# lc700x/desktop2stereo

Hardware: AMD Instinct MI355X
Metric: stereo frames/sec @1080p DepthAnything-v2-ViT-B (higher is better)
Workload: dtype bf16; 1 GPU; DepthAnything-v2-vitb bf16, 1920x1080 uint8 RGB noise frames, batch 1 per GPU, Depth Resolution 518 (model input 294x518), Full-SBS uint8 output 3840x1080, pred; parallelism=frame-sharded dp1, no data-path collective (each rank generates its own frames)

## Files before the change

### desktop2stereo_amd/csrc/core.cpp

```cpp
#include "common.h"

#include <atomic>
#include <cstdlib>

namespace d2s {

static thread_local std::string g_err;

void set_error(const std::string& msg) { g_err = msg; }

int hip_fail(hipError_t err, const char* what, const char* file, int line) {
    g_err = std::string("HIP error ") + hipGetErrorName(err) + " (" + hipGetErrorString(err) + ") in " + what +
            " at " + file + ":" + std::to_string(line);
    return D2S_E_HIP;
}

int env_int(const char* name, int dflt) {
    const char* v = getenv(name);
    return v ? atoi(v) : dflt;
}

static std::atomic<int> g_env_gen{1};
int env_generation() { return g_env_gen.load(std::memory_order_relaxed); }
int EnvInt::get() {
    const uint32_t g = (uint32_t)env_generation();
    const uint64_t c = cached.load(std::memory_order_relaxed);
    if ((uint32_t)(c >> 32) == g) return (int)(uint32_t)c;
    const int val = env_int(name, dflt);
    cached.store(((uint64_t)g << 32) | (uint32_t)val, std::memory_order_relaxed);
    return val;
}

int device_cu_count() {
    static const int n = [] { hipDeviceProp_t p; int d = 0; (void)hipGetDevice(&d); return hipGetDeviceProperties(&p, d) == hipSuccess ? p.multiProcessorCount : 256; }();
    return n;
}

}

extern "C" int d2s_debug_lds_poison(void) {
#ifdef D2S_LDS_POISON
    return 1;
#else
    return 0;
#endif
}
extern "C" int d2s_debug_reload_env(void) { return d2s::g_env_gen.fetch_add(1) + 1; }
extern "C" const char* d2s_last_error(void) { return d2s::g_err.c_str(); }
extern "C" int d2s_version(void) { return 132; }
```

### desktop2stereo_amd/csrc/gemm.hip

```cpp
#include "gemm_epi.h"
#include "linear_site.h"
#include <cstdio>
#include <deque>
#include <vector>

namespace d2s {

__device__ u32x4 d2s_zero_page[4];

#ifdef D2S_GLDS_TIMING
__device__ unsigned long long glds_timing[4096 * 8];
#define GL_STAMP(SLOT) { if (threadIdx.x == 0 && blockIdx.y == 0 && blockIdx.x < 4096) glds_timing[blockIdx.x * 8 + (SLOT)] = wall_clock64(); }
#else
#define GL_STAMP(SLOT) {}
#endif

__device__ __forceinline__ u32x4 relu_frag(u32x4 v, int, fp8_t) { return v; }
__device__ __forceinline__ u32x4 relu_frag(u32x4 v, int, bx3_t) { return v; }
__device__ __forceinline__ u32x4 relu_frag(u32x4 v, int floor_bits, float) {
    f32x4 x = __builtin_bit_cast(f32x4, v);
    float f = floor_bits == 0 ? 0.f : -3.0e38f;
    x = __builtin_elementwise_max(x, (f32x4){f, f, f, f});
    return __builtin_bit_cast(u32x4, x);
}

template <int N> __device__ __forceinline__ void wait_vmcnt() { asm volatile("s_waitcnt vmcnt(%0)" ::"n"(N) : "memory"); }

template <int CPR> __device__ __forceinline__ int swz_row(int r) { return CPR == 8 ? ((r >> 1) & 7) : (CPR == 4 ? ((r >> 1) & 3) : (r & 15)); }

static_assert(sizeof(GemmA) + sizeof(GemmEpi) + 8 >= KERNARG_WARM_BYTES, "KERNARG_WARM reads past the kernarg segment");
template <typename T, int BM, int BN, int WM, int WN, int NS, int CPR, int STG = 0>
__global__ void __launch_bounds__(64 * WM * WN)
gemm_glds_kernel(const T* __restrict__ W, const void* a_ptr, long a_lda, int M, int N, int K, int Kpad, int xn, GemmA a, GemmEpi e) {
    static_assert(STG == 0 || STG == 2 || (STG == 1 && NS == 2), "the register-staged variant uses two LDS stages");
    constexpr bool LEAN = STG == 2;
    constexpr bool BX3 = std::is_same<T, bx3_t>::value;
    static_assert(!BX3 || CPR == 8, "bf16x3 units are laid out for 128-byte K tiles");
    constexpr int CE = Prec<T>::CE;
    constexpr int BK = CPR * CE;
    constexpr int RPI = 64 / CPR;
    constexpr int NW = WM * WN;
    constexpr int AI = BM / (RPI * NW), BI = BN / (RPI * NW);
    constexpr int LPT = AI + BI;
    constexpr int FM = BM / WM / 16, FN = BN / WN / 16;
    constexpr int PD = NS - 1;
    constexpr int STAGE = (BM + BN) * CPR;
    __shared__ __attribute__((aligned(16))) u32x4 lds[NS * STAGE];
    KERNARG_WARM(kaw_)
    if constexpr (STG != 2) { KERNARG_WARM_END(kaw_) }
    D2S_POISON_LDS(lds, NS * STAGE)

    const int tid = threadIdx.x, lane = tid & 63;
    const int wid = __builtin_amdgcn_readfirstlane(tid >> 6);
    const int wave_m = wid / WN, wave_n = wid % WN;
    int tm_, tn_;
    GL_STAMP(0)
    if (!tile_of_block(blockIdx.x, (M + BM - 1) / BM, (N + BN - 1) / BN, xn, tm_, tn_)) return;
    const int bm0 = tm_ * BM, bn0 = tn_ * BN;
    static_assert((RPI * NW) % 16 == 0, "row swizzle must be invariant across a thread's instructions");
    static_assert(BM % (RPI * NW) == 0 && BN % (RPI * NW) == 0 && BM % (16 * WM) == 0 && BN % (16 * WN) == 0, "tile must split evenly over the waves");
    const int lrow = wid * RPI + lane / CPR;
    const int src_chunk = (lane % CPR) ^ swz_row<CPR>(lrow);
    const T* zero = (const T*)d2s_zero_page;

    const T* arow[AI];
    int aiy[AI], aix[AI];
    bool aok[AI];
    if constexpr (!LEAN)
#pragma unroll
    for (int i = 0; i < AI; ++i) {
        int m = bm0 + i * NW * RPI + lrow;
        aok[i] = m < M;
        int mm = aok[i] ? m : 0;
        if (a.mode == A_PLAIN) { arow[i] = (const T*)a.ptr + (long)mm * a.lda; aiy[i] = aix[i] = 0; }
        else {
            int ox = mm % a.Wo, oy = (mm / a.Wo) % a.Ho, b = mm / (a.Wo * a.Ho);
            aiy[i] = oy * a.stride - 1; aix[i] = ox * a.stride - 1;
            arow[i] = (const T*)a.ptr + (long)b * a.Hi * a.Wi * a.C;
        }
    }
    const T* wrow = W + (long)(bn0 + lrow) * Kpad + src_chunk * CE;
    const float inv_c = a.mode == A_CONV3 ? 1.0f / (float)a.C : 0.f;
    constexpr int ES = (int)sizeof(T);
    const __amdgpu_buffer_rsrc_t rsA = __builtin_amdgcn_make_buffer_rsrc(uniform_ptr(a_ptr), 0, (unsigned)((long)M * a_lda * ES), 0x00020000);
    const __amdgpu_buffer_rsrc_t rsW = __builtin_amdgcn_make_buffer_rsrc(uniform_ptr(W), 0, (unsigned)((long)((N + 255) / 256 * 256) * Kpad * ES), 0x00020000);
    unsigned voA[AI], voW[BI];
    if constexpr (STG != 1) {
        if (LEAN || a.buf) {
#pragma unroll
            for (int i = 0; i < AI; ++i) {
                const int m = bm0 + i * NW * RPI + lrow;
                voA[i] = m < M ? (unsigned)((long)m * a_lda * ES) + (unsigned)(src_chunk * 16) : 0x80000000u;
            }
#pragma unroll
            for (int i = 0; i < BI; ++i) voW[i] = (unsigned)((long)(bn0 + lrow + RPI * NW * i) * Kpad * ES) + (unsigned)(src_chunk * 16);
        }
    }
#define D2S_ISSUE_BUF(KT)                                                                                        \
    {                                                                                                            \
        u32x4* st_ = lds + ((KT) % NS) * STAGE;                                                                  \
        const int so_ = ((KT) + kt0) * (BK * ES);                                                                \
        _Pragma("unroll") for (int i = 0; i < AI; ++i) lds_dma16(rsA, st_ + (i * NW + wid) * 64, voA[i], so_);    \
        _Pragma("unroll") for (int i = 0; i < BI; ++i) lds_dma16(rsW, st_ + BM * CPR + (i * NW + wid) * 64, voW[i], so_); \
    }

    if constexpr (LEAN) {
        constexpr int kt0 = 0;
        const int nkt_ = (K + BK - 1) / BK;
#pragma unroll
        for (int t = 0; t < PD; ++t)
            if (t < nkt_) D2S_ISSUE_BUF(t)
        KERNARG_WARM_END(kaw_)
    }

    u32x4 stg[1][STG == 1 ? LPT : 1];
#define D2S_MOVE(S, IDX, SRC, DST)                                                                                \
    do {                                                                                                         \
        if constexpr (STG == 1) stg[S][IDX] = *(const u32x4*)(SRC);                                                 \
        else __builtin_amdgcn_global_load_lds((const __attribute__((address_space(1))) void*)(SRC),             \
                                              (__attribute__((address_space(3))) void*)(DST), 16, 0, 0);         \
    } while (0)
#define D2S_ISSUE_TILE(KT, S)                                                                                    \
    {                                                                                                            \
        u32x4* st_ = lds + ((KT) % NS) * STAGE;                                                                  \
        const int k_ = ((KT) + kt0) * BK + src_chunk * CE;                                                       \
        if (a.mode == A_PLAIN) {                                                                                 \
            _Pragma("unroll") for (int i = 0; i < AI; ++i) {                                                     \
                const T* s_ = (aok[i] && k_ < K) ? arow[i] + k_ : zero;                                          \
                D2S_MOVE(S, i, s_, st_ + (i * NW + wid) * 64);                                                    \
            }                                                                                                    \
        } else {                                                                                                 \
            int tap_ = (int)(((float)k_ + 0.5f) * inv_c);                                                        \
            int c0_ = k_ - tap_ * a.C;                                                                           \
            int ky_ = tap_ / 3, kx_ = tap_ - ky_ * 3;                                                            \
            _Pragma("unroll") for (int i = 0; i < AI; ++i) {                                                     \
                int iy_ = aiy[i] + ky_, ix_ = aix[i] + kx_;                                                      \
                bool ok_ = aok[i] && k_ < K && iy_ >= 0 && iy_ < a.Hi && ix_ >= 0 && ix_ < a.Wi;                 \
                const T* s_ = ok_ ? arow[i] + ((long)iy_ * a.Wi + ix_) * a.C + c0_ : zero;                       \
                D2S_MOVE(S, i, s_, st_ + (i * NW + wid) * 64);                                                    \
            }                                                                                                    \
        }                                                                                                        \
        _Pragma("unroll") for (int i = 0; i < BI; ++i)                                                           \
            D2S_MOVE(S, AI + i, wrow + (long)(RPI * NW * i) * Kpad + ((KT) + kt0) * BK, st_ + BM * CPR + (i * NW + wid) * 64); \
    }
    const int bx_row = (lane / CPR) * CPR, bx_sw = swz_row<CPR>(lrow);
    const int bx_hi = (bx_row + (((src_chunk >> 1) * 2) ^ bx_sw)) * 2 + (src_chunk & 1);
    const int bx_lo = (bx_row + (((src_chunk >> 1) * 2 + 1) ^ bx_sw)) * 2 + (src_chunk & 1);
#define D2S_STORE_STG(KT, S)                                                                                     \
    {                                                                                                            \
        u32x4* st_ = lds + ((KT) % NS) * STAGE;                                                                  \
        if constexpr (BX3) {                                                                                     \
            _Pragma("unroll") for (int i = 0; i < AI; ++i) {                                                     \
                f32x4 x_ = __builtin_bit_cast(f32x4, stg[S][i]);                                                 \
                if (a.relu) x_ = __builtin_elementwise_max(x_, (f32x4){0.f, 0.f, 0.f, 0.f});                     \
                uint2 h_, l_;                                                                                    \
                bx3_split4(x_, h_, l_);                                                                          \
                uint2* s2_ = (uint2*)(st_ + (i * NW + wid) * 64);                                                \
                s2_[bx_hi] = h_; s2_[bx_lo] = l_;                                                                \
            }                                                                                                    \
        } else {                                                                                                 \
            _Pragma("unroll") for (int i = 0; i < AI; ++i) st_[(i * NW + wid) * 64 + lane] = stg[S][i];          \
        }                                                                                                        \
        _Pragma("unroll") for (int i = 0; i < BI; ++i) st_[BM * CPR + (i * NW + wid) * 64 + lane] = stg[S][AI + i]; \
    }

    f32x4 acc[FM][FN];
#pragma unroll
    for (int i = 0; i < FM; ++i)
#pragma unroll
        for (int j = 0; j < FN; ++j) acc[i][j] = (f32x4){0.f, 0.f, 0.f, 0.f};

    const int nkt_all = (K + BK - 1) / BK;
    const int ksplit = LEAN ? 1 : (e.ksplit > 1 ? e.ksplit : 1);
    const int kt0 = (int)(((long)nkt_all * blockIdx.y) / ksplit);
    const int nkt = (int)(((long)nkt_all * (blockIdx.y + 1)) / ksplit) - kt0;
    const int fr = lane & 15, fg = lane >> 4;
    constexpr bool LN_ON = WN > 1;
    constexpr int LNS = LN_ON ? 4 : 1;
    float2 lnp[FM][LNS];
    if (LN_ON && e.ln_stats) {
#pragma unroll
        for (int i = 0; i < FM; ++i) {
            const int m = bm0 + wave_m * (BM / WM) + i * 16 + fr;
#pragma unroll
            for (int q = 0; q < LNS; ++q) {
                const int sl = fg + 4 * q;
                lnp[i][q] = (m < M && sl < e.ln_slots) ? ((const float2*)e.ln_stats)[(long)sl * (e.ln_M ? e.ln_M : M) + m] : make_float2(0.f, 0.f);
            }
        }
    }
#define D2S_COMPUTE(KT, RELU)                                                                                    \
    {                                                                                                            \
        const u32x4* A_l = lds + ((KT) % NS) * STAGE + (wave_m * (BM / WM)) * CPR;                               \
        const u32x4* B_l = lds + ((KT) % NS) * STAGE + BM * CPR + (wave_n * (BN / WN)) * CPR;                    \
        if constexpr (BX3) {                                                                                     \
             \
            const int cu_ = 2 * BX3_UNIT(fg);                                                                    \
            u32x4 fbh[FN], fbl[FN];                                                                              \
            _Pragma("unroll") for (int j = 0; j < FN; ++j) {                                                     \
                int r = j * 16 + fr; fbh[j] = B_l[r * CPR + (cu_ ^ swz_row<CPR>(r))]; fbl[j] = B_l[r * CPR + ((cu_ + 1) ^ swz_row<CPR>(r))]; \
            }                                                                                                    \
            _Pragma("unroll") for (int i = 0; i < FM; ++i) {                                                     \
                int r = i * 16 + fr;                                                                             \
                const u32x4 fah = A_l[r * CPR + (cu_ ^ swz_row<CPR>(r))], fal = A_l[r * CPR + ((cu_ + 1) ^ swz_row<CPR>(r))]; \
                _Pragma("unroll") for (int j = 0; j < FN; ++j) mma_bx3(acc[i][j], fbh[j], fbl[j], fah, fal);     \
            }                                                                                                    \
        } else {                                                                                                 \
        _Pragma("unroll") for (int ks = 0; ks < CPR / 4; ++ks) {                                                 \
                             \
                                            \
            u32x4 fb[FN];                                                                                        \
            _Pragma("unroll") for (int j = 0; j < FN; ++j) {                                                     \
                int r = j * 16 + fr; fb[j] = B_l[r * CPR + ((ks * 4 + fg) ^ swz_row<CPR>(r))];                   \
            }                                                                                                    \
            _Pragma("unroll") for (int i = 0; i < FM; ++i) {                                                     \
                int r = i * 16 + fr;                                                                             \
                u32x4 fa = A_l[r * CPR + ((ks * 4 + fg) ^ swz_row<CPR>(r))];                                     \
                if (RELU) fa = relu_frag(fa, 0, T());                                                            \
                _Pragma("unroll") for (int j = 0; j < FN; ++j) mma_chunk(acc[i][j], fb[j], fa, T());             \
            }                                                                                                    \
        }                                                                                                        \
        }                                                                                                        \
    }
#define D2S_K_LOOP(RELU)                                                                                         \
    if constexpr (STG == 1) {                                                                                    \
        for (int kt = 0; kt < nkt; ++kt) {                                                                       \
            __syncthreads();               \
            if (kt + 1 < nkt) D2S_STORE_STG(kt + 1, 0)                                                           \
            if (kt + 2 < nkt) D2S_ISSUE_TILE(kt + 2, 0)                                                          \
            D2S_COMPUTE(kt, RELU)                                                                                \
        }                                                                                                        \
    } else {                                                                                                     \
        for (int kt = 0; kt < nkt; ++kt) {                                                                       \
                          \
            if (kt + PD - 1 < nkt) wait_vmcnt<(PD - 1) * LPT>();                                                 \
            else wait_vmcnt<0>();                                                                                \
            __builtin_amdgcn_s_barrier();                                                                        \
            if (kt + PD < nkt) D2S_ISSUE_TILE(kt + PD, 0)                                                        \
            D2S_COMPUTE(kt, RELU)                                                                                \
        }                                                                                                        \
    }
    bool done_buf = false;
    if constexpr (STG != 1) {
        if (LEAN || a.buf) {
            if constexpr (!LEAN) {
#pragma unroll
                for (int t = 0; t < PD; ++t)
                    if (t < nkt) D2S_ISSUE_BUF(t)
            }
            GL_STAMP(1)
            for (int kt = 0; kt < nkt; ++kt) {
                if (kt + PD - 1 < nkt) wait_vmcnt<(PD - 1) * LPT>();
                else wait_vmcnt<0>();
                __builtin_amdgcn_s_barrier();
                if (kt == 0) { GL_STAMP(2) }
                if (kt + PD < nkt) D2S_ISSUE_BUF(kt + PD)
                D2S_COMPUTE(kt, 0)
            }
            done_buf = true;
        }
    }
    if constexpr (!LEAN)
    if (!done_buf) {
    if constexpr (STG == 1) {
        if (nkt > 0) { D2S_ISSUE_TILE(0, 0) D2S_STORE_STG(0, 0) }
        if (nkt > 1) D2S_ISSUE_TILE(1, 0)
    } else {
#pragma unroll
        for (int t = 0; t < PD; ++t)
            if (t < nkt) D2S_ISSUE_TILE(t, 0)
    }
    if (a.relu) { D2S_K_LOOP(1) } else { D2S_K_LOOP(0) }
    }
    GL_STAMP(3)
#undef D2S_ISSUE_BUF
#undef D2S_K_LOOP
#undef D2S_COMPUTE
#undef D2S_ISSUE_TILE
#undef D2S_STORE_STG
#undef D2S_MOVE

    if constexpr (WN == 1) {
        if (e.map == MAP_HEAD) {
            static_for<FM>([&](auto ic) {
                constexpr int i = decltype(ic)::value;
                const int m = bm0 + wave_m * (BM / WM) + i * 16 + fr;
                float s = 0.f;
                static_for<FN>([&](auto jc) {
                    constexpr int j = decltype(jc)::value;
                    const int n0 = j * 16 + fg * 4;
                    if (n0 < N) {
                        float b[4], w[4];
                        load4(e.bias + n0, b); load4(e.scale + n0, w);
                        s += fmaxf(acc[i][j][0] + b[0], 0.f) * w[0] + fmaxf(acc[i][j][1] + b[1], 0.f) * w[1] +
                             fmaxf(acc[i][j][2] + b[2], 0.f) * w[2] + fmaxf(acc[i][j][3] + b[3], 0.f) * w[3];
                    }
                });
                s += __shfl_xor(s, 16);
                s += __shfl_xor(s, 32);
                if (fg == 0 && m < M) ((float*)e.out)[m] = head_activation(s + e.head_b3, e.head_max_depth);
            });
            return;
        }
    }

    float2 ln_s[FM];
    float ln_cs[FN][4];
    if (LN_ON && e.ln_csum) {
#pragma unroll
        for (int j = 0; j < FN; ++j) {
            const int n0 = bn0 + wave_n * (BN / WN) + j * 16 + fg * 4;
            if (n0 < N) load4(e.ln_csum + n0, ln_cs[j]);
            else { ln_cs[j][0] = ln_cs[j][1] = ln_cs[j][2] = ln_cs[j][3] = 0.f; }
        }
    }
    constexpr bool PRE = STG == 2 && FM * FN <= 8;
    EpiCols cols[PRE ? FN : 1];
    if constexpr (PRE) {
#pragma unroll
        for (int j = 0; j < FN; ++j) {
            const int n0 = bn0 + wave_n * (BN / WN) + j * 16 + fg * 4;
            if (n0 < N) epi_cols_load(e, n0, cols[j]);
        }
    }
    float pre[PRE ? FM : 1][PRE ? FN : 1][4];
    const bool pre_on = PRE && ksplit == 1 && epi_res1_ahead(e);
    if constexpr (PRE) {
        if (pre_on) {
            static_for<FM>([&](auto ic) {
                constexpr int i = decltype(ic)::value;
                const int m = bm0 + wave_m * (BM / WM) + i * 16 + fr;
                static_for<FN>([&](auto jc) {
                    constexpr int j = decltype(jc)::value;
                    const int n0 = bn0 + wave_n * (BN / WN) + j * 16 + fg * 4;
                    if (m < M && n0 < N) epi_res1_load<T>(e, m, n0, pre[i][j]);
                });
            });
        }
    }
    static_for<FM>([&](auto ic) {
        constexpr int i = decltype(ic)::value;
        const int m = bm0 + wave_m * (BM / WM) + i * 16 + fr;
        float s1 = 0.f, s2 = 0.f;
        float ln_mean = 0.f, ln_rstd = 1.f;
        if (LN_ON && e.ln_csum) {
            float t1 = (lnp[i][0].x + lnp[i][1 % LNS].x) + (lnp[i][2 % LNS].x + lnp[i][3 % LNS].x);
            float t2 = (lnp[i][0].y + lnp[i][1 % LNS].y) + (lnp[i][2 % LNS].y + lnp[i][3 % LNS].y);
            t1 += __shfl_xor(t1, 16); t2 += __shfl_xor(t2, 16);
            t1 += __shfl_xor(t1, 32); t2 += __shfl_xor(t2, 32);
            ln_mean = t1 / (float)e.ln_dim;
            ln_rstd = rsqrtf(fmaxf(t2 / (float)e.ln_dim - ln_mean * ln_mean, 0.f) + e.ln_eps);
        }
        if (m < M) {
            static_for<FN>([&](auto jc) {
                constexpr int j = decltype(jc)::value;
                const int n0 = bn0 + wave_n * (BN / WN) + j * 16 + fg * 4;
                if (n0 < N) {
                    float v[4] = {acc[i][j][0], acc[i][j][1], acc[i][j][2], acc[i][j][3]};
                    if (ksplit > 1) store4(e.part + ((long)blockIdx.y * M + m) * N + n0, v);
                    else {
                        const bool ln = LN_ON && e.ln_csum != nullptr;
                        if (ln) {
                            if (e.deq) { float q[4]; load4(e.deq + n0, q); v[0] *= q[0]; v[1] *= q[1]; v[2] *= q[2]; v[3] *= q[3]; }
                            v[0] = ln_rstd * (v[0] - ln_mean * ln_cs[j][0]); v[1] = ln_rstd * (v[1] - ln_mean * ln_cs[j][1]);
                            v[2] = ln_rstd * (v[2] - ln_mean * ln_cs[j][2]); v[3] = ln_rstd * (v[3] - ln_mean * ln_cs[j][3]);
                        }
                        epilogue_dispatch<T>(e, m, n0, v, ln, PRE && pre_on ? pre[PRE ? i : 0][PRE ? j : 0] : nullptr, PRE ? &cols[PRE ? j : 0] : nullptr);
                        s1 += (v[0] + v[1]) + (v[2] + v[3]);
                        s2 += (v[0] * v[0] + v[1] * v[1]) + (v[2] * v[2] + v[3] * v[3]);
                    }
                }
            });
        }
        if (LN_ON && e.stats_out) {
            s1 += __shfl_xor(s1, 16); s2 += __shfl_xor(s2, 16);
            s1 += __shfl_xor(s1, 32); s2 += __shfl_xor(s2, 32);
            ln_s[i] = make_float2(s1, s2);
        }
    });
    if (LN_ON && e.stats_out) {
        float2* red = (float2*)lds;
        __syncthreads();
#pragma unroll
        for (int i = 0; i < FM; ++i)
            if (fg == 0) red[wave_n * BM + wave_m * (BM / WM) + i * 16 + fr] = ln_s[i];
        __syncthreads();
        for (int r = tid; r < BM; r += 64 * NW) {
            float2 t = red[r];
            for (int w = 1; w < WN; ++w) { t.x += red[w * BM + r].x; t.y += red[w * BM + r].y; }
            if (bm0 + r < M) ((float2*)e.stats_out)[(long)(bn0 / BN) * M + bm0 + r] = t;
        }
    }
#ifdef D2S_GLDS_TIMING
    asm volatile("s_waitcnt vmcnt(0)" ::: "memory");
    GL_STAMP(4)
#endif
}

template <typename T>
__global__ void __launch_bounds__(256)
splitk_reduce_kernel(GemmEpi e, int M, int N) {
    long idx = (long)blockIdx.x * blockDim.x + threadIdx.x;
    int n4 = N >> 2;
    if (idx >= (long)M * n4) return;
    int m = (int)(idx / n4), n0 = (int)(idx % n4) * 4;
    float v[4] = {0.f, 0.f, 0.f, 0.f};
    for (int s = 0; s < e.ksplit; ++s) {
        float p[4];
        load4(e.part + ((long)s * M + m) * N + n0, p);
        v[0] += p[0]; v[1] += p[1]; v[2] += p[2]; v[3] += p[3];
    }
    epilogue_dispatch<T>(e, m, n0, v);
}

template <typename T, int BN, int WM, int WN, int NS = 2>
__global__ void __launch_bounds__(64 * WM * WN)
conv3_halo_kernel(GemmA a, const T* __restrict__ W, int M, int N, int K, int Kpad, GemmEpi e, int xn) {
    KERNARG_WARM(kaw_)
    KERNARG_WARM_END(kaw_)
    constexpr int CE = Prec<T>::CE, CPR = 8, BK = CPR * CE, PD = NS - 1;
    constexpr int TW = 16, TH = 8, BM = TH * TW, HWD = TW + 2, HPX = (TH + 2) * HWD;
    constexpr int HCPP = 16;
    constexpr int NW = WM * WN, RPI = 64 / CPR;
    constexpr int BI = BN / (RPI * NW);
    static_assert(BI >= 1 && BM % (WM * 16) == 0 && BN % (WN * 16) == 0, "bad tile split");
    constexpr int FM = BM / WM / 16, FN = BN / WN / 16;
    constexpr int STAGE = BN * CPR;
    __shared__ __attribute__((aligned(16))) u32x4 lds[NS * STAGE + HPX * HCPP];
    D2S_POISON_LDS(lds, NS * STAGE + HPX * HCPP)
    u32x4* const halo = lds + NS * STAGE;

    const int tid = threadIdx.x, lane = tid & 63;
    const int wid = __builtin_amdgcn_readfirstlane(tid >> 6);
    const int wave_m = wid / WN, wave_n = wid % WN;
    const int tiles_x = (a.Wo + TW - 1) / TW, tiles_y = (a.Ho + TH - 1) / TH;
    const int nimg = M / (a.Ho * a.Wo);
    int tm_, tn_;
    if (!tile_of_block(blockIdx.x, nimg * tiles_y * tiles_x, (N + BN - 1) / BN, xn, tm_, tn_)) return;
    const int b = tm_ / (tiles_y * tiles_x), ty0 = ((tm_ / tiles_x) % tiles_y) * TH, tx0 = (tm_ % tiles_x) * TW;
    const int bn0 = tn_ * BN;
    const int cpp = a.C / CE, smask = cpp - 1;

    const int lrow = wid * RPI + lane / CPR;
    const int src_chunk = (lane % CPR) ^ swz_row<CPR>(lrow);
    const T* wrow = W + (long)(bn0 + lrow) * Kpad + src_chunk * CE;
#define D2S_ISSUE_W(KT)                                                                                               \
    {                                                                                                                 \
        u32x4* st_ = lds + ((KT) % NS) * STAGE;                                                                       \
        _Pragma("unroll") for (int i = 0; i < BI; ++i)                                                                \
            __builtin_amdgcn_global_load_lds((const __attribute__((address_space(1))) void*)(wrow + (long)(RPI * NW * i) * Kpad + (KT) * BK), \
                                             (__attribute__((address_space(3))) void*)(st_ + (i * NW + wid) * 64), 16, 0, 0);              \
    }
    const int nkt = K / BK;
#pragma unroll
    for (int t = 0; t < PD; ++t)
        if (t < nkt) D2S_ISSUE_W(t)
    conv_halo_fill<T, 64 * NW, 3>(a, b, ty0, tx0, HWD, HPX, cpp, tid, halo,
        [&](int p, int c) { return p * cpp + (c ^ (p & smask)); },
        [&](u32x4 v) { return a.relu ? relu_frag(v, 0, T()) : v; });
    f32x4 acc[FM][FN];
#pragma unroll
    for (int i = 0; i < FM; ++i)
#pragma unroll
        for (int j = 0; j < FN; ++j) acc[i][j] = (f32x4){0.f, 0.f, 0.f, 0.f};
    const int kpt = cpp / CPR;
    const int fr = lane & 15, fg = lane >> 4;
    int tap = 0, sub = 0;
    for (int kt = 0; kt < nkt; ++kt) {
        if (kt + PD - 1 < nkt) asm volatile("s_waitcnt vmcnt(%0) lgkmcnt(0)" ::"n"((PD - 1) * BI) : "memory");
        else asm volatile("s_waitcnt vmcnt(0) lgkmcnt(0)" ::: "memory");
        __builtin_amdgcn_s_barrier();
        if (kt + PD < nkt) D2S_ISSUE_W(kt + PD)
        const int ky = tap / 3, kx = tap - ky * 3, cb = sub * CPR;
        const u32x4* B_l = lds + (kt % NS) * STAGE + (wave_n * (BN / WN)) * CPR;
#pragma unroll
        for (int ks = 0; ks < CPR / 4; ++ks) {
            u32x4 fb[FN];
#pragma unroll
            for (int j = 0; j < FN; ++j) { int r = j * 16 + fr; fb[j] = B_l[r * CPR + ((ks * 4 + fg) ^ swz_row<CPR>(r))]; }
#pragma unroll
            for (int i = 0; i < FM; ++i) {
                const int p = (wave_m * FM + i + ky) * HWD + fr + kx;
                const u32x4 fa = halo[p * cpp + ((cb + ks * 4 + fg) ^ (p & smask))];
#pragma unroll
                for (int j = 0; j < FN; ++j) mma_chunk(acc[i][j], fb[j], fa, T());
            }
        }
        if (++sub == kpt) { sub = 0; ++tap; }
    }
#undef D2S_ISSUE_W
    const int nb = bn0 + wave_n * (BN / WN) + fg * 4;
    EpiCols cols[FN];
#pragma unroll
    for (int j = 0; j < FN; ++j)
        if (nb + j * 16 < N) epi_cols_load(e, nb + j * 16, cols[j]);
    conv_tile_epilogue<T, FM, FN>(a, e, acc, cols, b, ty0 + wave_m * FM, tx0 + fr, nb, N);
}

static inline bool buf_eligible(const GemmA& a, int M, int N, int K, int Kpad, int bk, size_t es) {
    return a.mode == A_PLAIN && !a.relu && K % bk == 0 && (long)M * a.lda * (long)es < (1L << 31) && (long)gemm_npad(N) * Kpad * (long)es < (1L << 31);
}

constexpr int SPLITK_GRID = 128;

static inline bool splitk_wanted(const GemmEpi& e, long tiles, int K, int bk) {
    return e.part && e.part_elems > 0 && !e.stats_out && tiles < SPLITK_GRID && cdiv(K, bk) >= 24;
}

static bool gemm_deep() {
    static EnvInt deep{"D2S_GEMM_DEEP", 1};
    return deep.get() != 0;
}

enum { TY_BF16 = 1, TY_E4M3 = 2, TY_F32 = 4, TY_BX3 = 8, TY_BEF = TY_BF16 | TY_E4M3 | TY_F32, TY_ALL = TY_BEF | TY_BX3 };
#define GLDS_INSTANCES(X)                                                                                                        \
                                                                                                   \
    X(G_256128, TY_BEF, 256,128,4,2,3,8,0)                                                                                       \
    X(G_128, TY_BEF, 128,128,2,2,4,8,0)                                                                                          \
    X(G_64, TY_BEF, 64,64,2,2,4,8,0)                                                                                             \
                      \
    X(G_3264, TY_ALL, 32,64,2,2,4,8,0)                                                                                           \
                             \
    X(G_1281288, TY_ALL, 128,128,2,4,2,8,0)                                                \
    X(G_641288, TY_ALL, 64,128,2,4,2,8,0)                                                                     \
    X(G_64648, TY_ALL, 64,64,4,2,2,8,0)                                                                       \
    X(G_256648, TY_BEF, 256,64,8,1,2,8,0)                                                         \
    X(G_128324, TY_BEF, 128,32,4,1,2,8,0)                                                                  \
          \
    X(G_964, TY_ALL, 64,64,2,2,2,8,1)                                                                                            \
    X(G_91288, TY_ALL, 128,128,4,2,2,8,1)                                                            \
    X(G_912832, TY_ALL, 128,32,4,1,2,8,1)                                                         \
    X(G_9256648, TY_ALL, 256,64,8,1,2,8,1)                                                                 \
// ... 24 lines not shown

static constexpr int glds_codes[][2] = {{256128, G_256128}, {128, G_128}, {64, G_64}, {3264, G_3264}, {1281288, G_1281288},
                                        {641288, G_641288}, {64648, G_64648}, {256648, G_256648}, {128324, G_128324}, {964, G_964},
                                        {91288, G_91288}, {912832, G_912832}, {9256648, G_9256648}};
static constexpr struct { int code, alias, auto_of, inst; } bx3_codes[] = {
    {93264, 3264, 3264, G_93264}, {964, 64, 64648, G_964}, {964128, 0, 641288, G_964128}, {91288, 128, 1281288, G_91288},
    {912832, 0, 912832, G_912832}, {9256648, 0, 9256648, G_9256648}};

#define HALO_INSTANCES(X) X(H_64, 64,4,2,4) X(H_128, 128,2,4,2)
enum {
#define X(ID, ...) ID,
    HALO_INSTANCES(X)
#undef X
};
static constexpr struct { int BN, WM, WN, NS; } halo_cfg[] = {
#define X(ID, ...) {__VA_ARGS__},
    HALO_INSTANCES(X)
#undef X
};
static const char* const halo_names[][4] = {
#define X(ID, ...) {"conv3_halo_kernel<bf16," #__VA_ARGS__ ">", nullptr, "conv3_halo_kernel<f32," #__VA_ARGS__ ">", nullptr},
    HALO_INSTANCES(X)
#undef X
};

static inline int type_index(int precision) {
    return precision == D2S_PREC_BF16 ? 0 : (precision == D2S_PREC_FP8_OPERANDS ? 1 : (precision == D2S_PREC_BF16X3 ? 3 : 2));
}
template <typename T> constexpr int type_bit() {
    return std::is_same<T, bf16_t>::value ? TY_BF16 : std::is_same<T, fp8_t>::value ? TY_E4M3 : std::is_same<T, bx3_t>::value ? TY_BX3 : TY_F32;
}

static int plan_fail(GemmPlan& p, int rc, const char* msg) { p.error = msg; return rc; }
static int glds_inst_of(int code) {
    for (const auto& c : glds_codes) if (c[0] == code) return c[1];
    return -1;
}

static int plan_glds(int inst, int precision, int tile, const GemmA& a, int M, int N, int K, int Kpad, const GemmEpi& e, GemmPlan& p) {
    const GldsCfg& c = glds_cfg[inst];
    const int es = (int)elem_size(precision), bk = c.CPR * (16 / es);
    p.family = GEMM_GLDS; p.inst = inst; p.name = glds_names[inst][type_index(precision)]; p.tile = tile; p.block = 64 * c.WM * c.WN;
    p.xn = pick_xn(cdiv(M, c.BM), cdiv(N, c.BN), c.BN, Kpad, es, p.grid);
    const int nkt = cdiv(K, bk);
    int ks = 1;
    if (c.STG != 2 && e.part && e.part_elems > 0 && !e.stats_out && (int)p.grid < SPLITK_GRID && nkt >= 24) {
        ks = nkt / 6; if (ks > 16) ks = 16;
        while (ks > 1 && (size_t)ks * M * N > e.part_elems) --ks;
    }
    static EnvInt sk_force{"D2S_SPLITK_FORCE", 0};
    if (sk_force.get() > 1 && c.STG != 2 && e.part && !e.stats_out && nkt >= sk_force.get() && (size_t)sk_force.get() * M * N <= e.part_elems) ks = sk_force.get();
    p.ksplit = ks; p.gridy = ks;
    if (ks > 1) { p.grid2 = cdiv((long)M * (N / 4), 256); return D2S_OK; }
    p.stats_slots = c.WN > 1 ? cdiv(N, c.BN) : 1 << 20;
    p.buf = c.STG != 1 && buf_eligible(a, M, N, K, Kpad, bk, es);
    return D2S_OK;
}

static int lean_of(int t, int precision, const GemmA& a, int M, int N, int K, int Kpad, const GemmEpi& e) {
    const int inst = t == 3264 ? G_L3264 : (t == 64648 ? G_L64648 : (t == 641288 ? G_L641288 : -1));
    if (inst < 0 || !gemm_deep() || !buf_eligible(a, M, N, K, Kpad, gemm_bk(precision), elem_size(precision))) return -1;
    const long tiles = (long)cdiv(M, glds_cfg[inst].BM) * cdiv(N, glds_cfg[inst].BN);
    return tiles <= 512 && !splitk_wanted(e, tiles, K, gemm_bk(precision)) ? inst : -1;
}

static int small_tile_of(int M, int N) {
    const long b128 = (long)cdiv(M, 128) * cdiv(N, 128), b64128 = (long)cdiv(M, 64) * cdiv(N, 128), b64 = (long)cdiv(M, 64) * cdiv(N, 64);
    if (b128 >= 400 && (N >= 1536 || b128 >= 900)) return 1281288;
    if (b64128 >= 280) return 641288;
    if (b64 >= 384) return 64648;
    return 3264;
}

static int auto_tile(int M, int N) {
    if (N <= 64) return (long)cdiv(M, 256) >= 224 ? (N <= 32 ? 912832 : 9256648) : 3264;
    return small_tile_of(M, N);
}

static bool plan_halo(int precision, const GemmA& a, int M, int N, int K, int Kpad, const GemmEpi& e, GemmPlan& p) {
    static EnvInt off{"D2S_NO_HALO", 0};
    if (off.get() || precision == D2S_PREC_FP8_OPERANDS) return false;
    const int es = (int)elem_size(precision), cpp = a.C * es / 16;
    if (a.mode != A_CONV3 || a.stride != 1 || a.Hi != a.Ho || a.Wi != a.Wo || (a.C * es) % 128 || cpp > 16 || (cpp & (cpp - 1))) return false;
    if (e.map != MAP_ROWS || e.rows_per_img || K != 9 * a.C || N <= 32) return false;
    const int nimg = M / (a.Ho * a.Wo);
    const long tiles_m = (long)nimg * cdiv(a.Ho, 8) * cdiv(a.Wo, 16);
    if (tiles_m * cdiv(N, 128) < 200 || (long)nimg * a.Ho * a.Wo != M) return false;
    const int inst = N <= 64 ? H_64 : H_128, bn = halo_cfg[inst].BN;
    p.family = GEMM_HALO; p.inst = inst; p.block = 64 * halo_cfg[inst].WM * halo_cfg[inst].WN; p.ups = a.ups;
    p.name = halo_names[inst][type_index(precision)];
    p.xn = pick_xn((int)tiles_m, cdiv(N, bn), bn, Kpad, es, p.grid);
    return true;
}

int gemm_pp_min_tiles() {
    static EnvInt v{"D2S_GEMM_PP", 100};
    return v.get();
}

int plan_gemm(int precision, int tile, const GemmA& a, int M, int N, int K, int Kpad, const GemmEpi& e, GemmPlan& p) {
    p = GemmPlan{};
    p.gridy = 1; p.ksplit = 1; p.buf = a.buf; p.stats_slots = -1;
    const int ce = 16 / (int)elem_size(precision);
    if (M <= 0 || N <= 0 || K <= 0 || (N & 3) || (K % ce) || Kpad % (2 * gemm_bk(precision)))
        return plan_fail(p, D2S_E_INVALID, "launch_gemm: bad dims (N % 4, K % chunk, Kpad % BK)");
    if (a.mode == A_PLAIN && (a.lda % ce)) return plan_fail(p, D2S_E_INVALID, "launch_gemm: lda not chunk aligned");
    if (a.mode == A_CONV3 && (a.C % ce)) return plan_fail(p, D2S_E_INVALID, "launch_gemm: conv channels not chunk aligned");
    if (precision == D2S_PREC_BF16X3) {
        if (e.deq || (e.out2 && !e.out2_bx3))
            return plan_fail(p, D2S_E_UNSUPPORTED, "launch_gemm: bf16x3 operands: no de-quantisation, raw-residual copies in the unit format only");
        if (a.bx3) {
            if (a.mode != A_PLAIN || a.relu) return plan_fail(p, D2S_E_UNSUPPORTED, "launch_gemm: a pre-split bf16x3 A operand must be a plain matrix");
            const int t = small_tile_of(M, N), lean = lean_of(t, precision, a, M, N, K, Kpad, e);
            return plan_glds(lean >= 0 ? lean : glds_inst_of(t), precision, t, a, M, N, K, Kpad, e, p);
        }
        if (tile == 256256) tile = 0;
        const int t = tile ? tile : auto_tile(M, N);
        for (const auto& c : bx3_codes)
            if (tile ? (tile == c.code || tile == c.alias) : t == c.auto_of) return plan_glds(c.inst, precision, tile ? tile : c.code, a, M, N, K, Kpad, e, p);
        return plan_fail(p, D2S_E_INVALID, "launch_gemm: bad tile code for bf16x3 operands");
    }
    if (tile == 256256) return plan_gemm_pp(precision, a, M, N, K, Kpad, e, p);
    if (precision == D2S_PREC_BF16 && a.mode == A_CONV3 && (tile == 0 || e.map == MAP_HEAD) && plan_conv3_halo2(a, M, N, K, Kpad, e, p)) return D2S_OK;
    if (a.ups) {
        if (precision == D2S_PREC_BF16 && tile == 0 && plan_halo(precision, a, M, N, K, Kpad, e, p)) return D2S_OK;
        return plan_fail(p, D2S_E_UNSUPPORTED, "launch_gemm: this launch cannot fold the up-sample into its loader (conv3_upsample_ok says when)");
    }
    if (precision == D2S_PREC_FP8_OPERANDS && (a.mode != A_PLAIN || a.relu)) return plan_fail(p, D2S_E_UNSUPPORTED, "launch_gemm: e4m3 operands are for plain linears");
    if (tile == 0 && plan_halo(precision, a, M, N, K, Kpad, e, p)) return D2S_OK;
    if (tile == 0 && sk_supported(precision, a, M, N, K, Kpad, e)) { plan_gemm_sk(a, M, N, K, p); return D2S_OK; }
    const int pp_min_tiles = gemm_pp_min_tiles();
    if (tile == 0 && pp_min_tiles > 0 && (long)cdiv(M, 256) * cdiv(N, 256) >= pp_min_tiles && pp_supported(precision, a, M, N, K, Kpad, e))
        return plan_gemm_pp(precision, a, M, N, K, Kpad, e, p);
    if (tile == 0) {
        tile = auto_tile(M, N);
        if (N > 64 && a.mode == A_CONV3 && K >= 4096 && (long)cdiv(M, 128) * cdiv(N, 128) >= 300) tile = 1281288;
    }
    if ((precision == D2S_PREC_BF16 || precision == D2S_PREC_FP8_OPERANDS) && !(e.part && e.ksplit > 1) && e.map != MAP_HEAD) {
        const int lean = lean_of(tile, precision, a, M, N, K, Kpad, e);
        if (lean >= 0) return plan_glds(lean, precision, tile, a, M, N, K, Kpad, e, p);
    }
    const int inst = glds_inst_of(tile);
    if (inst < 0) return plan_fail(p, D2S_E_INVALID, "launch_gemm: bad tile code");
    return plan_glds(inst, precision, tile, a, M, N, K, Kpad, e, p);
}

bool conv3_upsample_ok(int precision, int tile, const GemmA& a, int M, int N, int K, int Kpad, const GemmEpi& e) {
    static EnvInt no_ups{"D2S_NO_UPSFOLD", 0};
    if (no_ups.get() || precision != D2S_PREC_BF16 || a.mode != A_CONV3 || !a.ups || a.Hs < 2 || a.Ws < 2 || a.usy <= 0.f || a.usx <= 0.f) return false;
    GemmPlan p;
    return plan_gemm(precision, tile, a, M, N, K, Kpad, e, p) == D2S_OK && p.ups;
}

template <typename T>
static void launch_glds(const GemmPlan& p, const GemmA& a, const void* W, int M, int N, int K, int Kpad, const GemmEpi& e, hipStream_t st,
                        hipEvent_t stop) {
    const dim3 grid(p.grid, p.gridy), block(p.block);
    const hipEvent_t stop1 = p.grid2 ? nullptr : stop;
    if (p.family == GEMM_HALO) {
        if constexpr ((type_bit<T>() & (TY_BF16 | TY_F32)) != 0) switch (p.inst) {
#define X(ID, ...) case ID: hipLaunchKernelGGL((conv3_halo_kernel<T, __VA_ARGS__>), grid, block, 0, st, a, (const T*)W, M, N, K, Kpad, e, p.xn); break;
            HALO_INSTANCES(X)
#undef X
        }
        return;
    }
    switch (p.inst) {
#define X(ID, TY, ...) case ID: if constexpr (((TY) & type_bit<T>()) != 0) \
        D2S_LAUNCH_STOP(stop1, (gemm_glds_kernel<T, __VA_ARGS__>), grid, block, st, (const T*)W, a.ptr, a.lda, M, N, K, Kpad, p.xn, a, e); break;
        GLDS_INSTANCES(X)
#undef X
    }
    if (p.grid2) D2S_LAUNCH_STOP(stop, (splitk_reduce_kernel<T>), dim3(p.grid2), dim3(256), st, e, M, N);
}

static void note_kernel(const GemmPlan& p) { kernel_note() = KernelNote{p.name, p.tile, p.ksplit, p.tail}; }

int launch_gemm(int precision, int tile, const GemmA& a, const void* W, int M, int N, int K, int Kpad,
                const GemmEpi& e, hipStream_t st, hipEvent_t stop) {
    GemmPlan p;
    if (const int rc = plan_gemm(precision, tile, a, M, N, K, Kpad, e, p)) { set_error(p.error); return rc; }
    note_kernel(p);
    const bool in_launch = p.family == GEMM_GLDS || p.family == GEMM_PP;
    if (e.stats_slots && p.stats_slots >= 0) *e.stats_slots = p.stats_slots;
    GemmA a1 = a;
    a1.buf = p.buf;
    GemmEpi e1 = e;
    e1.ksplit = p.family == GEMM_GLDS ? p.ksplit : 1;
    switch (p.family) {
        case GEMM_CONV3: launch_conv3_halo2(p, a1, W, M, N, Kpad, e1, st); break;
        case GEMM_SK: launch_gemm_sk(p, a1, W, M, N, Kpad, e1, st); break;
        case GEMM_PP: if (const int rc = launch_gemm_pp(p, precision, a1, W, M, N, K, Kpad, e1, st, stop)) return rc; break;
        default: {
            const hipEvent_t ev = in_launch ? stop : nullptr;
            if (precision == D2S_PREC_BF16) launch_glds<bf16_t>(p, a1, W, M, N, K, Kpad, e1, st, ev);
            else if (precision == D2S_PREC_FP8_OPERANDS) launch_glds<fp8_t>(p, a1, W, M, N, K, Kpad, e1, st, ev);
            else if (precision == D2S_PREC_BF16X3) launch_glds<bx3_t>(p, a1, W, M, N, K, Kpad, e1, st, ev);
            else launch_glds<float>(p, a1, W, M, N, K, Kpad, e1, st, ev);
        }
    }
    D2S_CHECK_LAUNCH();
    if (stop && !in_launch) D2S_HIP(hipEventRecord(stop, st));
    return D2S_OK;
}

__global__ void cast_pad_kernel(const float* __restrict__ src, void* __restrict__ dst, int rows, int cols,
                                int rows_pad, int cols_pad, int prec) {
    long idx = (long)blockIdx.x * blockDim.x + threadIdx.x;
    if (idx >= (long)rows_pad * cols_pad) return;
    int c = (int)(idx % cols_pad), r = (int)(idx / cols_pad);
    float v = (r < rows && c < cols) ? src[(long)r * cols + c] : 0.f;
    if (prec == -D2S_PREC_BF16X3) {
        const bf16_t hi = f2bf(v), lo = f2bf(v - bf2f(hi));
        bf16_t* u = (bf16_t*)((char*)dst + ((long)r * cols_pad + (c & ~7)) * 4) + (c & 7);
        u[0] = hi; u[8] = lo;
    } else
    if (prec == D2S_PREC_BF16) ((bf16_t*)dst)[idx] = f2bf(v);
    else if (prec == D2S_PREC_FP8_OPERANDS) ((fp8_t*)dst)[idx] = f2e4m3(v);
    else ((float*)dst)[idx] = v;
}

}

using namespace d2s;

namespace d2s {

static thread_local KernelNote g_kernel_note = {};
KernelNote& kernel_note() { return g_kernel_note; }

namespace {
struct ProbeBuf {
    void* p = nullptr;
    ProbeBuf() = default;
    ProbeBuf(const ProbeBuf&) = delete;
    ProbeBuf& operator=(const ProbeBuf&) = delete;
    ~ProbeBuf() { if (p) (void)hipFree(p); }
};

int fetch_f32(std::vector<float>& h, const float* d, size_t n) {
    h.resize(n);
    D2S_HIP(hipMemcpy(h.data(), d, n * sizeof(float), hipMemcpyDeviceToHost));
    return D2S_OK;
}
int upload(ProbeBuf& buf, const void* h, size_t bytes) {
    D2S_HIP(hipMalloc(&buf.p, bytes));
    D2S_HIP(hipMemcpy(buf.p, h, bytes, hipMemcpyHostToDevice));
    return D2S_OK;
}

int alloc_splitk_ws(ProbeBuf& buf, size_t elems, hipStream_t st) {
    const size_t bytes = (elems + GEMM_PART_CTR_WORDS) * sizeof(float);
    D2S_HIP(hipMalloc(&buf.p, bytes));
    D2S_HIP(hipMemsetAsync(buf.p, 0, bytes, st));
    return D2S_OK;
}

std::string noted_kernel() {
    const KernelNote kn = kernel_note();
    std::string name = kn.name ? kn.name : "unrecorded";
    if (kn.name && !strncmp(kn.name, "gemm_glds_kernel", 16)) {
        name += " tile=" + std::to_string(kn.tile);
        if (kn.ksplit > 1) name += " splitk=" + std::to_string(kn.ksplit);
    } else if (kn.name && kn.tail != NOTE_TAIL_NONE) {
        static const char* const tails[4] = {"", "in-kernel", "two-launch", "row-split"};
        name += " ks=" + std::to_string(kn.ksplit) + " tail=" + tails[kn.tail];
    }
    return name;
}
}

}

extern "C" int d2s_gemm_probe(const float* A, const float* Wt, const float* bias, float* Cout, int M, int N, int K,
                              int precision, int tile, int iters, void* stream) {
    D2S_REQUIRE(A && Wt && Cout && M > 0 && N > 0 && K > 0 && (N % 4 == 0) && iters >= 1, "bad argument");
    D2S_REQUIRE(precision == D2S_PREC_BF16 || precision == D2S_PREC_FP32 || precision == D2S_PREC_FP8_OPERANDS || precision == D2S_PREC_BF16X3, "bad precision");
    hipStream_t st = (hipStream_t)stream;
    int bf = precision;
    int Kp = gemm_kpad(K, precision), Np = gemm_npad(N);
    size_t es = elem_size(precision);
    ProbeBuf dA, dW, dP;
    D2S_HIP(hipMalloc(&dA.p, (size_t)M * Kp * es));
    D2S_HIP(hipMalloc(&dW.p, (size_t)Np * Kp * es));
    hipLaunchKernelGGL(cast_pad_kernel, dim3(cdiv((long)M * Kp, 256)), dim3(256), 0, st, A, dA.p, M, K, M, Kp, bf);
    hipLaunchKernelGGL(cast_pad_kernel, dim3(cdiv((long)Np * Kp, 256)), dim3(256), 0, st, Wt, dW.p, N, K, Np, Kp, bf == D2S_PREC_BF16X3 ? -bf : bf);
    GemmA a = {};
    a.ptr = dA.p; a.mode = A_PLAIN; a.lda = Kp;
    GemmEpi e = {};
    e.out = Cout; e.out_type = OUT_F32; e.ldc = N; e.bias = bias;
    static EnvInt sk_force{"D2S_SPLITK_FORCE", 0};
    if (sk_force.get() > 1) {
        const size_t pe = (size_t)sk_force.get() * M * N;
        int rc = alloc_splitk_ws(dP, pe, st);
        if (rc != D2S_OK) return rc;
        e.part = (float*)dP.p; e.part_elems = pe;
    }
    int rc = D2S_OK;
    for (int i = 0; i < iters && rc == D2S_OK; ++i) rc = launch_gemm(precision, tile, a, dW.p, M, N, Kp, Kp, e, st);
    hipError_t err = hipStreamSynchronize(st);
    if (rc != D2S_OK) return rc;
    D2S_HIP(err);
    return D2S_OK;
}

extern "C" int d2s_conv3_probe(d2s_conv3_probe_params* p, void* stream) {
    D2S_REQUIRE(p && p->struct_size == sizeof(d2s_conv3_probe_params), "d2s_conv3_probe_params.struct_size must be sizeof(d2s_conv3_probe_params)");
    p->kernel[0] = 0;
    const int prec = p->precision, B = p->batch, C = p->C, N = p->N;
    D2S_REQUIRE(prec == D2S_PREC_BF16 || prec == D2S_PREC_FP32 || prec == D2S_PREC_BF16X3, "bad precision (bf16, fp32 or bf16x3)");
    D2S_REQUIRE(p->x && p->w && p->out && B > 0 && C > 0 && N > 0 && p->Hs > 0 && p->Ws > 0 && p->Hi > 0 && p->Wi > 0, "bad argument");
    D2S_REQUIRE(p->stride == 1 || p->stride == 2, "stride must be 1 or 2");
    const bool ups = p->Hs != p->Hi || p->Ws != p->Wi;
    D2S_REQUIRE(!ups || p->stride == 1, "a folded up-sample needs stride 1");
    D2S_REQUIRE(!p->map_head || (p->w3 && !p->res && p->act == 0 && p->stride == 1), "map_head: w3 needed; no residual, no act, stride 1");
    hipStream_t st = (hipStream_t)stream;
    const int Ho = (p->Hi + 2 - 3) / p->stride + 1, Wo = (p->Wi + 2 - 3) / p->stride + 1;
    const long M = (long)B * Ho * Wo, nsrc = (long)B * p->Hs * p->Ws;
// ... 270 lines not shown
```

Measured before the change: 955.7 stereo frames/s.

## Keep GEMM weight fragments in registers for lean bf16 tiles, deepen A pipeline

Adds a WREG variant of the lean bf16 GLDS GEMM kernel. Weight fragments are loaded straight from global memory into registers with buffer loads, and only the A tile is staged in LDS through a deeper pipeline (9 or 16 stages). Waves are remapped so that each wave owns distinct N columns. This cuts LDS traffic and the LDS footprint for W and allows more prefetch depth, at the cost of extra VGPRs and uncoalesced per-wave W reads. The variant is enabled by default for three tile instances when there is no split-K and no stats output.

New measurement: 794.8 stereo frames/s. 16.8% lower.

```diff
diff --git a/desktop2stereo_amd/csrc/core.cpp b/desktop2stereo_amd/csrc/core.cpp
--- a/desktop2stereo_amd/csrc/core.cpp
+++ b/desktop2stereo_amd/csrc/core.cpp
@@ -47,4 +47,4 @@
 }
 extern "C" int d2s_debug_reload_env(void) { return d2s::g_env_gen.fetch_add(1) + 1; }
 extern "C" const char* d2s_last_error(void) { return d2s::g_err.c_str(); }
-extern "C" int d2s_version(void) { return 132; }
+extern "C" int d2s_version(void) { return 133; }
diff --git a/desktop2stereo_amd/csrc/gemm.hip b/desktop2stereo_amd/csrc/gemm.hip
--- a/desktop2stereo_amd/csrc/gemm.hip
+++ b/desktop2stereo_amd/csrc/gemm.hip
@@ -29,11 +29,21 @@
 template <int CPR> __device__ __forceinline__ int swz_row(int r) { return CPR == 8 ? ((r >> 1) & 7) : (CPR == 4 ? ((r >> 1) & 3) : (r & 15)); }
 
 static_assert(sizeof(GemmA) + sizeof(GemmEpi) + 8 >= KERNARG_WARM_BYTES, "KERNARG_WARM reads past the kernarg segment");
-template <typename T, int BM, int BN, int WM, int WN, int NS, int CPR, int STG = 0>
-__global__ void __launch_bounds__(64 * WM * WN)
+#ifndef D2S_WREG_REMAP
+#define D2S_WREG_REMAP 1
+#endif
+struct WregCfg { int NS, PW; };
+constexpr WregCfg wreg_cfg(int BM, int BN) { return BM == 32 ? WregCfg{16, 8} : (BN == 64 ? WregCfg{9, 8} : WregCfg{9, 6}); }
+constexpr int wreg_wn(int BN, int NW) { return D2S_WREG_REMAP ? (BN / 16 < NW ? BN / 16 : NW) : 0; }
+template <typename T, int BM, int BN, int WM_, int WN_, int NS_, int CPR, int STG = 0, bool WREG = false>
+__global__ void __launch_bounds__(64 * WM_ * WN_)
 gemm_glds_kernel(const T* __restrict__ W, const void* a_ptr, long a_lda, int M, int N, int K, int Kpad, int xn, GemmA a, GemmEpi e) {
-    static_assert(STG == 0 || STG == 2 || (STG == 1 && NS == 2), "the register-staged variant uses two LDS stages");
+    static_assert(STG == 0 || STG == 2 || (STG == 1 && NS_ == 2), "the register-staged variant uses two LDS stages");
     constexpr bool LEAN = STG == 2;
+    static_assert(!WREG || (LEAN && std::is_same<T, bf16_t>::value), "W in registers: the lean bf16 instantiations");
+    constexpr int WN = WREG && wreg_wn(BN, WM_ * WN_) ? wreg_wn(BN, WM_ * WN_) : WN_, WM = WM_ * WN_ / WN;
+    constexpr bool REMAP = WN != WN_;
+    constexpr int NS = WREG ? wreg_cfg(BM, BN).NS : NS_;
     constexpr bool BX3 = std::is_same<T, bx3_t>::value;
     static_assert(!BX3 || CPR == 8, "bf16x3 units are laid out for 128-byte K tiles");
     constexpr int CE = Prec<T>::CE;
@@ -44,7 +54,11 @@
     constexpr int LPT = AI + BI;
     constexpr int FM = BM / WM / 16, FN = BN / WN / 16;
     constexpr int PD = NS - 1;
-    constexpr int STAGE = (BM + BN) * CPR;
+    constexpr int STAGE = (WREG ? BM : BM + BN) * CPR;
+    constexpr int PW = WREG ? wreg_cfg(BM, BN).PW : 1;
+    constexpr int WL = (CPR / 4) * FN;
+    static_assert(!WREG || (PD >= PW && PD * AI + PW * WL < 64), "WREG: W(kt) is the youngest request of tile kt; vmcnt has 6 bits");
+    static_assert(!WREG || NS * STAGE * 16 <= 80 * 1024, "WREG: two blocks per CU");
     __shared__ __attribute__((aligned(16))) u32x4 lds[NS * STAGE];
     KERNARG_WARM(kaw_)
     if constexpr (STG != 2) { KERNARG_WARM_END(kaw_) }
@@ -103,13 +117,42 @@
         _Pragma("unroll") for (int i = 0; i < AI; ++i) lds_dma16(rsA, st_ + (i * NW + wid) * 64, voA[i], so_);    \
         _Pragma("unroll") for (int i = 0; i < BI; ++i) lds_dma16(rsW, st_ + BM * CPR + (i * NW + wid) * 64, voW[i], so_); \
     }
+    u32x4 wq[PW][CPR / 4][FN];
+    unsigned voQ[FN];
+    if constexpr (WREG) {
+#pragma unroll
+        for (int j = 0; j < FN; ++j)
+            voQ[j] = (unsigned)((long)(bn0 + wave_n * (BN / WN) + j * 16 + (lane & 15)) * Kpad * ES) + (unsigned)((lane >> 4) * 16);
+    }
+#define D2S_WREG_A(KT, NKT)                                                                                      \
+    {                                                                                                            \
+        u32x4* st_ = lds + ((KT) % NS) * STAGE;                                                                  \
+        const unsigned past_ = (KT) < (NKT) ? 0u : 0x80000000u;                                                  \
+        _Pragma("unroll") for (int i = 0; i < AI; ++i) lds_dma16(rsA, st_ + (i * NW + wid) * 64, voA[i] | past_, (KT) * (BK * ES)); \
+    }
+#define D2S_WREG_W(KT, NKT, S)                                                                                   \
+    {                                                                                                            \
+        const unsigned past_ = (KT) < (NKT) ? 0u : 0x80000000u;                                                  \
+        _Pragma("unroll") for (int ks = 0; ks < CPR / 4; ++ks)                                                   \
+            _Pragma("unroll") for (int j = 0; j < FN; ++j)                                                       \
+                wq[S][ks][j] = __builtin_bit_cast(u32x4, __builtin_amdgcn_raw_buffer_load_b128(rsW, voQ[j] | past_, (KT) * (BK * ES) + ks * 64, 0)); \
+    }
 
     if constexpr (LEAN) {
         constexpr int kt0 = 0;
         const int nkt_ = (K + BK - 1) / BK;
+        if constexpr (WREG) {
+            static_for<PD>([&](auto tc) {
+                constexpr int t = decltype(tc)::value;
+                D2S_WREG_A(t, nkt_)
+                if constexpr (t >= PD - PW) D2S_WREG_W(t - (PD - PW), nkt_, t - (PD - PW))
+                asm volatile("" ::: "memory");
+            });
+        } else {
 #pragma unroll
         for (int t = 0; t < PD; ++t)
             if (t < nkt_) D2S_ISSUE_BUF(t)
+        }
         KERNARG_WARM_END(kaw_)
     }
 
@@ -249,6 +292,43 @@
                     if (t < nkt) D2S_ISSUE_BUF(t)
             }
             GL_STAMP(1)
+            if constexpr (WREG) {
+                constexpr int WREG_VMCNT = (PW - 1) * (AI + WL);
+#define D2S_WREG_COMPUTE(KT, S)                                                                                  \
+                {                                                                                                \
+                    const u32x4* A_l = lds + ((KT) % NS) * STAGE + (wave_m * (BM / WM)) * CPR;                   \
+                    _Pragma("unroll") for (int ks = 0; ks < CPR / 4; ++ks)                                       \
+                        _Pragma("unroll") for (int i = 0; i < FM; ++i) {                                         \
+                            const int r = i * 16 + fr;                                                           \
+                            const u32x4 fa = A_l[r * CPR + ((ks * 4 + fg) ^ swz_row<CPR>(r))];                   \
+                            _Pragma("unroll") for (int j = 0; j < FN; ++j) mma_chunk(acc[i][j], wq[S][ks][j], fa, T()); \
+                        }                                                                                        \
+                }
+                int kb = 0;
+                for (; kb + PW <= nkt; kb += PW) {
+                    static_for<PW>([&](auto sc) {
+                        constexpr int s = decltype(sc)::value;
+                        const int kt = kb + s;
+                        wait_vmcnt<WREG_VMCNT>();
+                        __builtin_amdgcn_s_barrier();
+                        if (kt == 0) { GL_STAMP(2) }
+                        D2S_WREG_A(kt + PD, nkt)
+                        D2S_WREG_COMPUTE(kt, s)
+                        D2S_WREG_W(kt + PW, nkt, s)
+                    });
+                }
+                static_for<PW - 1>([&](auto uc) {
+                    constexpr int u = decltype(uc)::value;
+                    if (kb + u < nkt) {
+                        wait_vmcnt<(PW - 1 - u) * (AI + WL)>();
+                        __builtin_amdgcn_s_barrier();
+                        if (kb + u == 0) { GL_STAMP(2) }
+                        D2S_WREG_COMPUTE(kb + u, u)
+                    }
+                });
+                wait_vmcnt<0>();
+#undef D2S_WREG_COMPUTE
+            } else
             for (int kt = 0; kt < nkt; ++kt) {
                 if (kt + PD - 1 < nkt) wait_vmcnt<(PD - 1) * LPT>();
                 else wait_vmcnt<0>();
@@ -378,6 +458,7 @@
             ln_s[i] = make_float2(s1, s2);
         }
     });
+    if constexpr (!REMAP)
     if (LN_ON && e.stats_out) {
         float2* red = (float2*)lds;
         __syncthreads();
@@ -708,6 +789,16 @@
     return plan_gemm(precision, tile, a, M, N, K, Kpad, e, p) == D2S_OK && p.ups;
 }
 
+constexpr int WREG_KEPT = 7;
+constexpr int wreg_bit(int inst) {
+    const int bit = inst == G_L3264 ? 0 : (inst == G_L64648 ? 1 : (inst == G_L641288 ? 2 : -1));
+    return bit >= 0 && (WREG_KEPT >> bit & 1) ? bit : -1;
+}
+static int gemm_wreg() {
+    static EnvInt v{"D2S_GEMM_WREG", WREG_KEPT};
+    return v.get();
+}
+
 template <typename T>
 static void launch_glds(const GemmPlan& p, const GemmA& a, const void* W, int M, int N, int K, int Kpad, const GemmEpi& e, hipStream_t st,
                         hipEvent_t stop) {
@@ -720,6 +811,18 @@
 #undef X
         }
         return;
+    }
+    if constexpr (std::is_same<T, bf16_t>::value) {
+        const int bit = wreg_bit(p.inst);
+        if (bit >= 0 && (gemm_wreg() >> bit & 1) && p.buf && p.ksplit == 1 && !e.stats_out) {
+            switch (p.inst) {
+#define X(ID, TY, ...) case ID: if constexpr (wreg_bit(ID) >= 0) \
+                D2S_LAUNCH_STOP(stop1, (gemm_glds_kernel<T, __VA_ARGS__, true>), grid, block, st, (const T*)W, a.ptr, a.lda, M, N, K, Kpad, p.xn, a, e); break;
+                GLDS_INSTANCES(X)
+#undef X
+            }
+            return;
+        }
     }
     switch (p.inst) {
 #define X(ID, TY, ...) case ID: if constexpr (((TY) & type_bit<T>()) != 0) \
```
